# DINT-NSDI24/DINT

Measured on NVIDIA H100. Metric: committed txns/sec (lock_fasst), higher is better.
Workload: dtype u32

## Files before the change

### dint_b200/csrc/engine.cu

```cuda
#include <cmath>
#include <cstdio>
#include <cstdlib>
#include <cstring>
#include <string>
#include <algorithm>
#include <chrono>
#include <type_traits>
#include <vector>
#include <cerrno>
#include <fcntl.h>
#include <sys/stat.h>
#include <unistd.h>

#include "../../include/dint_b200.h"
#include "kernels.cuh"
#include "route.cuh"
#include "kv.cuh"
#include "clients.cuh"
#include "txn_clients.cuh"
#include "image.cuh"
#include "reshard.cuh"
#include "rebuild.cuh"

using namespace dint;

static thread_local std::string g_last_error;
static int set_err(int code, const char* what, cudaError_t ce = cudaSuccess) {
  char buf[1024];
  if (ce != cudaSuccess) snprintf(buf, sizeof buf, "%s: %s", what, cudaGetErrorString(ce));
  else snprintf(buf, sizeof buf, "%s", what);
  g_last_error = buf;
  return code;
}
template <typename... Args>
static int set_errf(int code, const char* fmt, Args... args) {
  char buf[1024];
  snprintf(buf, sizeof buf, fmt, args...);
  return set_err(code, buf);
}
#define CU(call)                                                              \
  do {                                                                        \
    cudaError_t _e = (call);                                                  \
    if (_e != cudaSuccess) return set_err(_e == cudaErrorMemoryAllocation ? DINT_ENOMEM : DINT_EIO, #call, _e); \
  } while (0)

static const uint32_t kMsgSize[DINT_NUM_KINDS] = {6, 9, 53, 53, 55, 23};
static const uint32_t kLogEntry[DINT_NUM_KINDS] = {0, 0, 56, 0, 64, 32};
static const uint32_t kValSize[DINT_NUM_KINDS] = {0, 0, 0, 40, 40, 8};

constexpr int kExecStoreEbpf = DINT_NUM_KINDS;
constexpr int kExecTatpEbpf = DINT_NUM_KINDS + 1;
constexpr int kExecSmallbankEbpf = DINT_NUM_KINDS + 2;

template <class F>
static int with_kind(int kind, F&& f) {
  switch (kind) {
    case DINT_LOCK2PL: return f(std::integral_constant<int, K_LOCK2PL>{});
    case DINT_FASST: return f(std::integral_constant<int, K_FASST>{});
    case DINT_LOG: return f(std::integral_constant<int, K_LOG>{});
    case DINT_STORE: return f(std::integral_constant<int, K_STORE>{});
    case DINT_TATP: return f(std::integral_constant<int, K_TATP>{});
    case DINT_SMALLBANK: return f(std::integral_constant<int, K_SMALLBANK>{});
    case kExecStoreEbpf: return f(std::integral_constant<int, K_STORE_EBPF>{});
    case kExecTatpEbpf: return f(std::integral_constant<int, K_TATP_EBPF>{});
    case kExecSmallbankEbpf: return f(std::integral_constant<int, K_SMALLBANK_EBPF>{});
  }
  return set_err(DINT_EINVAL, "bad kind");
}

struct StepTarget {
  uint32_t seg_tiles;
  uint64_t seg_resp[kMaxShards];
  bool pad_ok;
  const uint32_t* skip;
};

enum { KT_CLASSIFY = 0, KT_LOGSCAN, KT_APPLY, KT_ORDERED, KT_LOAD, KT_NUM };
static const char* kKernelNames[KT_NUM] = {"k_classify", "k_log_scan", "k_apply", "k_ordered", "k_kv_load"};

struct EvPair { cudaEvent_t a, b; int which; };
constexpr int kHostBufs = 4;
struct HostRing {
  struct Buf { uint8_t* p = nullptr; size_t cap = 0; };
  Buf in[kHostBufs], aux[kHostBufs], out[kHostBufs];
  cudaEvent_t h2d[kHostBufs]{}, released[kHostBufs]{}, ready[kHostBufs]{}, d2h[kHostBufs]{};
  cudaStream_t s_in = nullptr, s_out = nullptr;
  uint32_t sets = 0;
};

struct dint_engine {
  int kind = 0;
  int device = 0;
  dint_cfg cfg{};
  uint32_t msg = 0;
  uint32_t chunk = 0;
  uint32_t max_tiles = 0;
  bool has_log = false;
  Ctx ctx{};
  std::vector<void*> allocs;
  cudaStream_t stream = nullptr;
  HostRing ring;
  uint32_t host_chunk = 0;
  bool plain_launches = false;
  uint32_t host_min_slice = 0;
  bool host_ramp_up = true;
  unsigned long long* h_counters = nullptr;
  unsigned long long* h_kvcnt = nullptr;
  cudaEvent_t ev_kvcnt = nullptr;
  int coop_grid = 0;
  int sms = 0;
  int grid_classify = 0, grid_apply = 0;
  uint32_t smem_stage = 0;
  uint64_t total_groups = 0;
  uint32_t* d_flags[2] = {nullptr, nullptr};
  uint32_t* d_grp[2] = {nullptr, nullptr};
  uint64_t chunk_seq = 0;
  uint32_t prev_n = 0;
  bool ord_pending = false;
  uint8_t* ord_resp = nullptr;
  const uint8_t* ord_req = nullptr;
  uint32_t ord_tile0 = 0;
  uint32_t smem_classify = 0;
  uint32_t* d_nc = nullptr;
  uint32_t* d_route = nullptr;
  uint32_t route_tiles = 0;
  uint32_t* d_route2 = nullptr;
  uint32_t route_desc_tiles = 0, route_seq = 0;
  int grid_route = 0;
  uint8_t* hot_arena = nullptr;
  size_t hot_bytes = 0;
  bool use_window = false;
  cudaAccessPolicyWindow window{};
  dint_stats stats{};
  uint32_t profiling = 0;
  std::vector<EvPair> ev_pool;
  size_t ev_used = 0;
  double kt_ms[KT_NUM] = {0};
  uint64_t kt_n[KT_NUM] = {0};
  KvHost kv[kMaxTables];
};

static bool sbe_on(const dint_engine* e) { return e->kind == DINT_SMALLBANK && e->ctx.ecache; }
static int exec_kind(const dint_engine* e) {
  return e->ctx.tchain ? kExecTatpEbpf : sbe_on(e) ? kExecSmallbankEbpf : e->ctx.ecache ? kExecStoreEbpf : e->kind;
}

template <typename T>
static int dalloc(dint_engine* e, T** p, size_t count, bool zero = true) {
  size_t bytes = count * sizeof(T);
  if (bytes == 0) bytes = sizeof(T);
  void* q = nullptr;
  CU(cudaMalloc(&q, bytes));
  e->allocs.push_back(q);
  if (zero) CU(cudaMemsetAsync(q, 0, bytes, e->stream));
  *p = (T*)q;
  return DINT_OK;
}

static int prof_flush(dint_engine* e) {
  for (size_t i = 0; i < e->ev_used; i++) {
    float ms = 0;
    CU(cudaEventSynchronize(e->ev_pool[i].b));
    CU(cudaEventElapsedTime(&ms, e->ev_pool[i].a, e->ev_pool[i].b));
    e->kt_ms[e->ev_pool[i].which] += ms;
    e->kt_n[e->ev_pool[i].which]++;
  }
  e->ev_used = 0;
  return DINT_OK;
}
struct ProfScope {
  dint_engine* e; cudaStream_t s; EvPair* p = nullptr;
  ProfScope(dint_engine* e_, cudaStream_t s_, int which) : e(e_), s(s_) {
    e->stats.kernel_launches++;
    if (!((e->profiling >> which) & 1u)) return;
    if (e->ev_used == e->ev_pool.size()) {
      if (e->ev_pool.size() >= 8192) { prof_flush(e); }
      else {
        EvPair np{}; cudaEventCreate(&np.a); cudaEventCreate(&np.b);
        e->ev_pool.push_back(np);
      }
    }
    p = &e->ev_pool[e->ev_used++];
    p->which = which;
    cudaEventRecord(p->a, s);
  }
  ~ProfScope() { if (p) cudaEventRecord(p->b, s); }
};

template <typename... Args>
static cudaError_t launch_ex(dint_engine* e, void (*kern)(Args...), int grid, int block, size_t smem, cudaStream_t s,
                             bool coop, Args... args) {
  cudaLaunchConfig_t cfg{};
  cfg.gridDim = dim3(grid < 1 ? 1 : grid);
  cfg.blockDim = dim3(block);
  cfg.dynamicSmemBytes = smem;
  cfg.stream = s;
  cudaLaunchAttribute at[3];
  int na = 0;
  if (coop) { at[na].id = cudaLaunchAttributeCooperative; at[na].val.cooperative = 1; na++; }
  if (e->use_window) { at[na].id = cudaLaunchAttributeAccessPolicyWindow; at[na].val.accessPolicyWindow = e->window; na++; }
  cfg.attrs = at;
  cfg.numAttrs = na;
  return cudaLaunchKernelEx(&cfg, kern, args...);
}

template <int KIND>
static int launch_chunk_t(dint_engine* e, const Ctx& c, cudaStream_t s) {
  {
    ProfScope ps(e, s, KT_CLASSIFY);
    int want = (int)c.n_tiles, clr = (int)((c.prev_n + 4 * kTile - 1) / (4 * kTile));
    if (clr > want) want = clr;
    int grid = (want < e->grid_classify && !c.ord_pending) ? want : e->grid_classify;
    if (c.n == 0 && e->sms > 0 && grid > 8 * e->sms) grid = 8 * e->sms;
    CU(launch_ex(e, k_classify<KIND>, grid, kTile, e->smem_classify, s, false, c));
  }
  if (c.n == 0) { CU(cudaGetLastError()); return DINT_OK; }
  if (kHasLog<KIND>) {
    ProfScope ps(e, s, KT_LOGSCAN);
    k_log_scan<<<1, kThreads, 0, s>>>(c);
  }
  {
    ProfScope ps(e, s, KT_APPLY);
    int grid = (int)c.n_tiles < e->grid_apply ? (int)c.n_tiles : e->grid_apply;
    CU(launch_ex(e, k_apply<KIND>, grid, kTile, e->smem_stage, s, false, c));
  }
  if ((KIND == K_TATP || KIND == K_TATP_EBPF) && c.n > c.ring_n) {
    int grid = (int)((c.ring_n + kThreads - 1) / kThreads);
    if (e->sms > 0 && grid > 4 * e->sms) grid = 4 * e->sms;
    k_log_vals<<<grid, kThreads, 0, s>>>(c);
    e->stats.kernel_launches++;
  }
  if (KIND != K_LOG) {
    ProfScope ps(e, s, KT_ORDERED);
    Ctx f = c;
    f.nc_ord = c.nc_cur;
    f.ord_resp = c.resp;
    f.ord_req = c.req;
    f.ord_tile0 = c.tile0;
    f.coop_launch = e->plain_launches ? 0u : 1u;
    int g3 = e->coop_grid;
    if (e->plain_launches && e->sms > 0) {
      const int per = g3 / e->sms;
      g3 = (per > 1 ? per - 1 : 1) * e->sms;
    }
    CU(launch_ex(e, k_ordered<KIND>, g3, kThreads, 0, s, !e->plain_launches, f));
  }
  CU(cudaGetLastError());
  return DINT_OK;
}

static int launch_chunk(dint_engine* e, const Ctx& c, cudaStream_t s) {
  return with_kind(exec_kind(e), [&](auto k) { return launch_chunk_t<decltype(k)::value>(e, c, s); });
}

template <int KIND>
static int grids_for(dint_engine* e) {
  int per_sm = 0, sms = 0;
  CU(cudaDeviceGetAttribute(&sms, cudaDevAttrMultiProcessorCount, e->device));
  e->sms = sms;
  e->grid_route = 4 * sms;
  e->smem_stage = Stage<Wire<KIND>::MSG>::N * Stage<Wire<KIND>::MSG>::BYTES;
  if (e->smem_stage > 48 * 1024) {
    CU(cudaFuncSetAttribute(k_classify<KIND>, cudaFuncAttributeMaxDynamicSharedMemorySize, (int)e->smem_stage));
    CU(cudaFuncSetAttribute(k_apply<KIND>, cudaFuncAttributeMaxDynamicSharedMemorySize, (int)e->smem_stage));
  }
  e->smem_classify = e->smem_stage;
  if (KIND != K_LOG && (kTile / 32) * OrdSlice<KIND>::BYTES > e->smem_classify) e->smem_classify = (kTile / 32) * OrdSlice<KIND>::BYTES;
  CU(cudaOccupancyMaxActiveBlocksPerMultiprocessor(&per_sm, k_classify<KIND>, kTile, e->smem_classify));
  if (per_sm < 1) return set_err(DINT_EIO, "k_classify cannot be resident");
  e->grid_classify = per_sm * sms;
  CU(cudaOccupancyMaxActiveBlocksPerMultiprocessor(&per_sm, k_apply<KIND>, kTile, e->smem_stage));
  if (per_sm < 1) return set_err(DINT_EIO, "k_apply cannot be resident");
  e->grid_apply = per_sm * sms;
  if (KIND == K_LOG) { e->coop_grid = 1; return DINT_OK; }
  CU(cudaOccupancyMaxActiveBlocksPerMultiprocessor(&per_sm, k_ordered<KIND>, kThreads, 0));
  if (per_sm < 1) return set_err(DINT_EIO, "k_ordered cannot be resident");
  if (per_sm > 4) per_sm = 4;
  e->coop_grid = per_sm * sms;
  return DINT_OK;
}

static void fill_chunk_ctx(dint_engine* e, Ctx& c, const StepTarget* tgt) {
  const int cur = (int)(e->chunk_seq & 1);
  c.grp = e->d_grp[cur];
  c.grp_prev = e->d_grp[cur ^ 1];
  c.flags = e->d_flags[cur];
  c.flags_prev = e->d_flags[cur ^ 1];
  c.prev_n = e->prev_n;
  c.clear_set = (uint64_t)(c.flags_mask + 1) / 256 <= e->prev_n ? 1u : 0u;
  c.nc_cur = e->d_nc + 4 * cur;
  c.nc_ord = e->d_nc + 4 * (cur ^ 1);
  c.ord_pending = e->ord_pending ? 1u : 0u;
  c.ord_resp = e->ord_resp;
  c.ord_req = e->ord_req;
  c.ord_tile0 = e->ord_tile0;
  if (tgt) {
    c.seg_tiles = tgt->seg_tiles;
    c.pad_ok = tgt->pad_ok ? 1u : 0u;
    c.skip = tgt->skip;
    for (int i = 0; i < kMaxShards; i++) c.seg_resp[i] = tgt->seg_resp[i];
  }
}

static int submit_chunk(dint_engine* e, const uint8_t* req, uint32_t n, uint8_t* resp, cudaStream_t s, uint32_t tile0 = 0,
                        const StepTarget* tgt = nullptr) {
  Ctx c = e->ctx;
  c.n = n;
  c.n_tiles = (n + kTile - 1) / kTile;
  c.req = req;
  c.resp = resp;
  c.tile0 = tile0;
  fill_chunk_ctx(e, c, tgt);
  int rc = launch_chunk(e, c, s);
// ... 185 lines not shown
  }
  e->route_seq = e->route_seq % 255u + 1u;
  if (e->route_seq == 1)
    CU(cudaMemsetAsync(e->d_route2, 0, 64 + (size_t)(e->route_desc_tiles + e->route_desc_tiles / 32 + 1) * 4 * sizeof(unsigned long long), s));
  RouteArgs b = a;
  b.done = e->d_route2;
  b.ticket = e->d_route2 + 1;
  b.totals = e->d_route2 + 4;
  b.desc = (unsigned long long*)(e->d_route2 + 16);
  b.gdesc = b.desc + (size_t)e->route_desc_tiles * 4;
  b.seq = e->route_seq;
  if (CUDART_VERSION >= 11000 && RT::SMEM > 48 * 1024) CU(cudaFuncSetAttribute(k_route_dispatch<KIND>, cudaFuncAttributeMaxDynamicSharedMemorySize, (int)RT::SMEM));
  int grid = (int)b.n_tiles < e->grid_route ? (int)b.n_tiles : e->grid_route;
  if (grid < 1) grid = 1;
  k_route_dispatch<KIND><<<grid, kThreads, RT::SMEM, s>>>(e->ctx, b);
  CU(cudaGetLastError());
  return DINT_OK;
}
template <int MSG>
static int route_combine_t(dint_engine* e, const RouteArgs& a, cudaStream_t s) {
  using RT = RTile<MSG>;
  int grid = (int)a.n_tiles;
  if (grid > e->grid_route) grid = e->grid_route;
  k_route_combine<MSG><<<grid, kThreads, RT::SMEM, s>>>(a);
  CU(cudaGetLastError());
  return DINT_OK;
}
static uint32_t route_tile_records(const dint_engine* e) { return e->msg <= 12 ? kThreads * 8u : (uint32_t)kThreads; }

extern "C" {

uint32_t dint_msg_size(int kind) { return (kind >= 0 && kind < DINT_NUM_KINDS) ? kMsgSize[kind] : 0; }
uint32_t dint_log_entry_size(int kind) { return (kind >= 0 && kind < DINT_NUM_KINDS) ? kLogEntry[kind] : 0; }
const char* dint_last_error(void) { return g_last_error.c_str(); }
uint64_t dint_test_fasthash64(uint64_t x, int len) { return len == 4 ? fasthash64_u32((uint32_t)x) : fasthash64_u64(x); }
uint32_t dint_test_fastmod(uint64_t n, uint32_t d) { FastMod f = make_fastmod(d); return fast_mod(n, f); }
int dint_test_rebuild_source(uint64_t key, uint32_t G, uint32_t lost_mask) {
  return G == 0 || G > kMaxShards ? -1 : rebuild_source((uint32_t)(key % G), G, lost_mask);
}
uint32_t dint_test_host_slices(uint64_t n, uint32_t min_slice, uint32_t max_slice, int ramp_up, uint32_t* out, uint32_t cap) {
  HostSlices sched(n, min_slice, max_slice, ramp_up != 0);
  uint32_t k = 0;
  for (uint32_t cn; (cn = sched.next()) != 0; k++)
    if (k < cap) out[k] = cn;
  return k;
}

void dint_default_cfg(int kind, dint_cfg* cfg) {
  memset(cfg, 0, sizeof *cfg);
  cfg->lock_slots = 36000000u;
  cfg->log_ring = 1000000u;
  cfg->subs_sizing = (kind == DINT_TATP) ? 7000000u : 2000000u;
  cfg->subs_populate = cfg->subs_sizing;
  cfg->accts_sizing = 24000000u;
  cfg->accts_populate = cfg->accts_sizing;
  cfg->n_shards = 1;
  cfg->shard_id = 0;
  cfg->chunk = 1u << 20;
}

void* dint_host_alloc(size_t bytes) {
  void* p = nullptr;
  if (cudaHostAlloc(&p, bytes ? bytes : 1, cudaHostAllocDefault) != cudaSuccess) { cudaGetLastError(); return nullptr; }
  return p;
}
void dint_host_free(void* p) { if (p) cudaFreeHost(p); }

void dint_destroy(dint_engine* e) {
  if (!e) return;
  cudaSetDevice(e->device);
  cudaDeviceSynchronize();
  for (void* p : e->allocs) cudaFree(p);
  if (e->d_route) cudaFree(e->d_route);
  if (e->d_route2) cudaFree(e->d_route2);
  if (e->h_counters) cudaFreeHost(e->h_counters);
  if (e->h_kvcnt) cudaFreeHost(e->h_kvcnt);
  if (e->ev_kvcnt) cudaEventDestroy(e->ev_kvcnt);
  for (auto& ep : e->ev_pool) { cudaEventDestroy(ep.a); cudaEventDestroy(ep.b); }
  HostRing& R = e->ring;
  for (int i = 0; i < kHostBufs; i++) {
    for (HostRing::Buf* b : {&R.in[i], &R.aux[i], &R.out[i]}) cudaFree(b->p);
    for (cudaEvent_t ev : {R.h2d[i], R.released[i], R.ready[i], R.d2h[i]}) if (ev) cudaEventDestroy(ev);
  }
  for (cudaStream_t s : {e->stream, R.s_in, R.s_out}) if (s) cudaStreamDestroy(s);
  delete e;
}

static int create_impl(dint_engine* e) {
  const dint_cfg& cf = e->cfg;
  Ctx& c = e->ctx;
  CU(cudaSetDevice(e->device));
  CU(cudaStreamCreateWithFlags(&e->stream, cudaStreamNonBlocking));
  HostRing& R = e->ring;
  for (cudaStream_t* s : {&R.s_in, &R.s_out}) CU(cudaStreamCreateWithFlags(s, cudaStreamNonBlocking));
  for (int i = 0; i < kHostBufs; i++)
    for (cudaEvent_t* ev : {&R.h2d[i], &R.released[i], &R.ready[i], &R.d2h[i]}) CU(cudaEventCreateWithFlags(ev, cudaEventDisableTiming));
  c.n_shards = cf.n_shards;
  c.shard_id = cf.shard_id;
  c.shard_div = make_fastmod(cf.n_shards);
  c.slot_mod = make_fastmod(cf.lock_slots);
  c.ring_n = cf.log_ring ? cf.log_ring : 1;

  uint64_t groups = 0;
  auto local_groups = [&](uint64_t global) { return (global + cf.n_shards - 1) / cf.n_shards; };
  int rc;
  switch (e->kind) {
    case DINT_LOCK2PL:
      groups = local_groups(cf.lock_slots);
      if ((rc = dalloc(e, &c.cnt2, groups))) return rc;
      break;
    case DINT_FASST:
      groups = local_groups(cf.lock_slots);
      if ((rc = dalloc(e, &c.ver, groups))) return rc;
      break;
    case DINT_LOG:
      groups = 0;
      break;
    default:
      if ((rc = kv_create_tables(e->kind, cf, c, e->kv, &groups,
                                 [&](void** p, size_t bytes) -> int {
                                   uint8_t* q = nullptr;
                                   int r = dalloc(e, &q, bytes);
                                   *p = q;
                                   return r;
                                 },
                                 (cf.flags & DINT_CFG_TATP_EBPF) != 0)))
        return rc == DINT_EINVAL ? set_err(rc, "bad KV configuration") : rc;
      break;
  }
  e->total_groups = groups;
  if (groups >= 0xffffffffULL) return set_err(DINT_EINVAL, "too many groups");
  if ((cf.flags & DINT_CFG_LOCK_HOLDER_KEYS) && (rc = dalloc(e, &c.holder, groups))) return rc;
  if (cf.flags & DINT_CFG_STORE_EBPF_MASK) {
    c.ecache_variant = (cf.flags & DINT_CFG_STORE_EBPF_MASK) >> 1;
    if ((rc = dalloc(e, &c.ecache, groups * kEcSetBytes))) return rc;
    if ((rc = dalloc(e, &c.ecache_stats, EC_NSTATS))) return rc;
  }
  if (cf.flags & DINT_CFG_TATP_EBPF) {
    const uint64_t buckets = groups / 4;
    for (uint32_t t = 0; t < c.n_tables; t++) c.tbkt_mod[t] = make_fastmod(e->kv[t].hash_size);
    c.tpool_cap = (uint32_t)(buckets + buckets / 2 + 4096);
    if ((rc = dalloc(e, &c.ecache, buckets * kEcSetBytes))) return rc;
    if ((rc = dalloc(e, &c.ecache_stats, EC_NSTATS_TATP))) return rc;
    if ((rc = dalloc(e, &c.tchain, buckets))) return rc;
    if ((rc = dalloc(e, &c.tpool, (size_t)c.tpool_cap * kTeEntBytes))) return rc;
    if ((rc = dalloc(e, &c.tpool_top, 1))) return rc;
  }
  if (cf.flags & DINT_CFG_SMALLBANK_EBPF) {
    for (uint32_t t = 0; t < c.n_tables; t++) c.tbkt_mod[t] = make_fastmod(e->kv[t].hash_size);
    if ((rc = dalloc(e, &c.ecache, groups / 4 * kSbeSetBytes))) return rc;
    if ((rc = dalloc(e, &c.ecache_stats, SBE_NSTATS))) return rc;
  }
  {
    uint32_t fl = 25;
    while (fl > 10 && (1ULL << (fl - 1)) >= groups * 2 + 2048) fl--;
    c.flags_mask = (1u << fl) - 1;
    const size_t set_bytes = (size_t)4 << (fl - 3);
    const size_t lock_bytes = (e->kind == DINT_FASST) ? (((groups + 31) / 32) * 4 + 255) / 256 * 256 : 0;
    e->hot_bytes = 2 * set_bytes + lock_bytes;
    if ((rc = dalloc(e, &e->hot_arena, e->hot_bytes))) return rc;
    e->d_flags[0] = (uint32_t*)e->hot_arena;
    e->d_flags[1] = (uint32_t*)(e->hot_arena + set_bytes);
    if (lock_bytes) c.lockbits = (uint32_t*)(e->hot_arena + 2 * set_bytes);
    int max_persist = 0, max_win = 0;
    cudaDeviceGetAttribute(&max_persist, cudaDevAttrMaxPersistingL2CacheSize, e->device);
    cudaDeviceGetAttribute(&max_win, cudaDevAttrMaxAccessPolicyWindowSize, e->device);
    if (max_persist > 0 && max_win > 0) {
      size_t want = e->hot_bytes < (size_t)max_persist ? e->hot_bytes : (size_t)max_persist;
      if (cudaDeviceSetLimit(cudaLimitPersistingL2CacheSize, want) == cudaSuccess) {
        e->window.base_ptr = e->hot_arena;
        e->window.num_bytes = e->hot_bytes < (size_t)max_win ? e->hot_bytes : (size_t)max_win;
        e->window.hitRatio = (float)((double)want / (double)e->window.num_bytes > 1.0 ? 1.0 : (double)want / (double)e->window.num_bytes);
        e->window.hitProp = cudaAccessPropertyPersisting;
        e->window.missProp = cudaAccessPropertyStreaming;
        e->use_window = true;
// ... 2725 lines not shown
```

### dint_b200/csrc/kernels.cuh

```cuda
#pragma once
#include <cooperative_groups.h>
#include "engine.cuh"

namespace dint {
namespace cg = cooperative_groups;

DINT_D uint32_t lane_id() { return threadIdx.x & 31; }
DINT_D uint32_t warp_id() { return threadIdx.x >> 5; }

DINT_D uint32_t tile_rank(bool flag, uint32_t* scratch, uint32_t& total) {
  uint32_t bal = __ballot_sync(0xffffffffu, flag);
  uint32_t in_warp = __popc(bal & ((1u << lane_id()) - 1u));
  if (lane_id() == 0) scratch[warp_id()] = __popc(bal);
  __syncthreads();
  uint32_t off = 0, tot = 0;
#pragma unroll
  for (int w = 0; w < kTile / 32; w++) {
    uint32_t v = scratch[w];
    if (w < (int)warp_id()) off += v;
    tot += v;
  }
  __syncthreads();
  total = tot;
  return off + in_warp;
// ... 106 lines not shown
}
template <int KIND>
__global__ void __launch_bounds__(kThreads) k_route_owner(const Ctx c, const uint8_t* req, uint32_t n, uint8_t* owner) {
  const uint32_t i = blockIdx.x * kThreads + threadIdx.x;
  if (i < n) owner[i] = (uint8_t)route_owner_of<KIND>(c, req + (size_t)i * Wire<KIND>::MSG);
}

constexpr int kMaxShards = 8;
__global__ void __launch_bounds__(kThreads) k_exact_count(const uint8_t* owner, uint32_t n, uint32_t world, uint32_t* tilecnt) {
  __shared__ uint32_t cnt[kMaxShards];
  if (threadIdx.x < kMaxShards) cnt[threadIdx.x] = 0;
  __syncthreads();
  const uint32_t i = blockIdx.x * kThreads + threadIdx.x;
  const uint32_t o = i < n ? owner[i] : 0xffu;
  const uint32_t peers = __match_any_sync(0xffffffffu, o);
  if (o < world && (int)lane_id() == __ffs(peers) - 1) atomicAdd(&cnt[o], (uint32_t)__popc(peers));
  __syncthreads();
  if (threadIdx.x < world) tilecnt[(size_t)threadIdx.x * gridDim.x + blockIdx.x] = cnt[threadIdx.x];
}
__global__ void __launch_bounds__(kThreads) k_exact_scan(uint32_t* tilecnt, uint32_t n_tiles, uint32_t* totals) {
  __shared__ uint32_t wsum[kThreads / 32];
  uint32_t* row = tilecnt + (size_t)blockIdx.x * n_tiles;
  const uint32_t total = cta_exclusive_scan<uint32_t>(row, row, n_tiles, 0u, wsum);
  if (threadIdx.x == 0) totals[blockIdx.x] = total;
}
template <int MSG>
__global__ void __launch_bounds__(kThreads) k_exact_scatter(const uint8_t* req, const uint8_t* owner, uint32_t n, uint32_t world,
                                                            const uint32_t* tilebase, const uint32_t* totals, uint8_t* out,
                                                            uint32_t* perm) {
  __shared__ uint32_t wcnt[kThreads / 32][kMaxShards];
  const uint32_t i = blockIdx.x * kThreads + threadIdx.x;
  if (threadIdx.x < (kThreads / 32) * kMaxShards) ((uint32_t*)wcnt)[threadIdx.x] = 0;
  __syncthreads();
  const uint32_t o = i < n ? owner[i] : 0xffu;
  const uint32_t peers = __match_any_sync(0xffffffffu, o);
  const uint32_t before = __popc(peers & ((1u << lane_id()) - 1u));
  if (o < world && before == 0) wcnt[warp_id()][o] = __popc(peers);
  __syncthreads();
  if (o < world) {
    uint32_t pos = tilebase[(size_t)o * gridDim.x + blockIdx.x] + before;
    for (uint32_t w = 0; w < warp_id(); w++) pos += wcnt[w][o];
    for (uint32_t q = 0; q < o; q++) pos += totals[q];
    copy_record<MSG>(out + (size_t)pos * MSG, req + (size_t)i * MSG);
    perm[pos] = i;
  }
}
struct PeerPtrs { uint64_t p[kMaxShards]; };

__global__ void k_p2p_signal(PeerPtrs sig, uint32_t world, uint32_t me, uint32_t epoch) {
  if (threadIdx.x < world) {
    __threadfence_system();
    volatile uint32_t* flag = (volatile uint32_t*)sig.p[threadIdx.x] + me;
    asm volatile("st.release.sys.global.u32 [%0], %1;" ::"l"(flag), "r"(epoch) : "memory");
  }
}
constexpr uint32_t kSigOverflow = 0x80000000u;
__global__ void k_p2p_wait(const uint32_t* my_sig, uint32_t world, uint32_t epoch, uint32_t* timeout, uint32_t* bad) {
  if (threadIdx.x < world) {
    const long long t0 = clock64();
    uint32_t v;
    do {
      asm volatile("ld.acquire.sys.global.u32 %0, [%1];" : "=r"(v) : "l"(my_sig + threadIdx.x) : "memory");
      if (clock64() - t0 > 8000000000LL) { atomicExch(timeout, 1u); break; }
    } while ((int32_t)((v & ~kSigOverflow) - epoch) < 0);
    if (bad && (v & kSigOverflow) && (v & ~kSigOverflow) == epoch) atomicCAS(bad, 0u, epoch);
  }
  __syncthreads();
  __threadfence_system();
}

template <int MSG>
__global__ void __launch_bounds__(kThreads) k_exact_unpermute(const uint8_t* sorted, const uint32_t* perm, uint32_t n, uint8_t* out) {
  const uint32_t pos = blockIdx.x * kThreads + threadIdx.x;
  if (pos >= n) return;
  const uint32_t idx = perm[pos];
  if (idx == 0xffffffffu) return;
  copy_record<MSG>(out + (size_t)idx * MSG, sorted + (size_t)pos * MSG);
}

template <int KIND> struct OrdSlice {
  static constexpr uint32_t BYTES = kBucketCap * (FastReplay<KIND>::ok ? (8 + 8 + 4) : 8);
};
template <int KIND> DINT_D void ordered_buckets(const Ctx& c, uint8_t* scratch);

template <int KIND>
__global__ void __launch_bounds__(kTile) k_classify(const Ctx c) {
  using W = Wire<KIND>;
  constexpr uint32_t NS = Stage<W::MSG>::N;
  extern __shared__ __align__(128) uint8_t smem[];
  __shared__ uint64_t full[kStages];
  __shared__ uint32_t scratch[kTile / 32];
  if (c.skip && __ldcg(c.skip)) return;
  if (threadIdx.x == 0) {
    for (int s = 0; s < kStages; s++) mbar_init(&full[s], 1);
    if (blockIdx.x == 0) { c.nc_cur[0] = 0; c.nc_cur[1] = 0; c.nc_ord[2] = 0; }
  }
  __syncthreads();
  const bool do_ord = c.ord_pending && c.nc_ord[0] != 0 && c.nc_ord[1] == 0;
  const bool ord_first = (blockIdx.x & 1u) != 0;
  if (do_ord && ord_first) {
    ordered_buckets<KIND>(c, smem);
    __syncthreads();
  }
  const TileIter it = tile_iter(c.n_tiles);
  if (threadIdx.x == 0)
    for (uint32_t i = 0; i < NS && i < it.n_my; i++) issue_tile_load<W::MSG>(c, smem, full, it, i);

  if (c.clear_set) {
    uint4* f4 = (uint4*)c.flags_prev;
    const uint32_t n4 = (c.flags_mask + 1) / 32;
    for (uint32_t i = blockIdx.x * kTile + threadIdx.x; i < n4; i += gridDim.x * kTile) f4[i] = make_uint4(0, 0, 0, 0);
  }
  for (uint32_t i = blockIdx.x * kTile + threadIdx.x; !c.clear_set && i < c.prev_n; i += 4 * gridDim.x * kTile) {
    uint32_t g[4];
#pragma unroll
    for (int u = 0; u < 4; u++) {
      const uint32_t j = i + u * gridDim.x * kTile;
      g[u] = j < c.prev_n ? __ldcg(&c.grp_prev[j]) : kNoGroup;
    }
#pragma unroll
    for (int u = 0; u < 4; u++)
      if (g[u] != kNoGroup) c.flags_prev[flag_word(c, g[u])] = 0;
  }

  uint32_t pend_old = 0, pend_test = 0, pend_sh = 0;
  uint32_t* pend_w = nullptr;
  bool saw_writer = false;
  for (uint32_t i = 0; it.has(i); i++) {
    if (threadIdx.x == 0 && i && i + NS - 1 < it.n_my) issue_tile_load<W::MSG>(c, smem, full, it, i + NS - 1);
    uint32_t first, cnt;
    const uint8_t* tile = acquire_tile<W::MSG>(c, smem, full, it, i, first, cnt);
    const bool valid = threadIdx.x < cnt;
    bool is_log = false;
    uint32_t new_old = 0, new_test = 0, new_sh = 0;
    uint32_t* new_w = nullptr;
    if (valid) {
      const uint8_t* rec = tile + threadIdx.x * W::MSG;
      TypeInfo ti = (c.pad_ok && rec[W::TYPE] == kPadType) ? TypeInfo{0, false, false} : type_info<KIND>(rec);
      uint32_t g = kNoGroup;
      if (!ti.invalid && ti.mask) {
        g = key_info<KIND>(c, rec).grp;
        if (g != kNoGroup) {
          uint32_t* w = &c.flags[flag_word(c, g)];
          const uint32_t sh = flag_shift(g);
          if (ti.mask == C_RA) {
            atomicOr(w, F_R << sh);
          } else {
            const uint32_t bits = ((ti.mask & C_RA) ? F_R : 0u) | ((ti.mask & C_WA) ? F_WA : 0u) | ((ti.mask & C_WL) ? F_WL : 0u);
            saw_writer = true;
            new_old = atomicOr(w, bits << sh);
            new_test = ((ti.mask & C_WA) ? F_WA : 0u) | ((ti.mask & C_WL) ? F_WL : 0u);
            new_w = w;
            new_sh = sh;
          }
        }
      }
      c.grp[first + threadIdx.x] = g;
      is_log = !ti.invalid && ti.is_log;
    }
    if (pend_w && ((pend_old >> pend_sh) & pend_test)) atomicOr(pend_w, F_W2 << pend_sh);
    pend_old = new_old; pend_test = new_test; pend_sh = new_sh; pend_w = new_w;
    if (kHasLog<KIND>) {
      uint32_t total;
      (void)tile_rank(is_log, scratch, total);
      if (threadIdx.x == 0) c.log_tilecnt[it.tile(i)] = total;
    } else {
      __syncthreads();
    }
  }
  if (pend_w && ((pend_old >> pend_sh) & pend_test)) atomicOr(pend_w, F_W2 << pend_sh);
  if (__syncthreads_or(saw_writer ? 1 : 0) && threadIdx.x == 0) atomicOr(&c.nc_cur[2], 1u);
  if (do_ord && !ord_first) {
    __syncthreads();
    ordered_buckets<KIND>(c, smem);
  }
}

__global__ void __launch_bounds__(kThreads) k_log_scan(const Ctx c) {
  if (c.skip && __ldcg(c.skip)) return;
  __shared__ uint32_t wsum[kThreads / 32];
  const unsigned long long end =
      cta_exclusive_scan<unsigned long long>(c.log_tilecnt, c.log_tilebase, c.n_tiles, threadIdx.x == 0 ? c.log_total[0] : 0ull, wsum);
  if (threadIdx.x == 0) {
    c.log_total[1] = end;
    c.log_total[0] = end;
  }
}

__global__ void __launch_bounds__(kThreads) k_log_vals(const Ctx c) {
  using W = Wire<K_TATP>;
  if (c.skip && __ldcg(c.skip)) return;
  const unsigned long long base = c.log_tilebase[0], end = c.log_total[1];
  if (end - base <= c.ring_n) return;
  for (unsigned long long ord = end - c.ring_n + blockIdx.x * kThreads + threadIdx.x; ord < end; ord += (unsigned long long)gridDim.x * kThreads) {
    if (c.log_src[ord - base] & 1u) continue;
    for (unsigned long long o = ord; o >= base + c.ring_n;) {
      o -= c.ring_n;
      const uint32_t s = c.log_src[o - base];
      if (s & 1u) {
        const uint8_t* src = c.req + (size_t)(s >> 1) * W::MSG + W::VAL;
        uint8_t* e = c.ring + (size_t)(ord % c.ring_n) * W::LOGENT + 16;
        for (int b = 0; b < 40; b++) e[b] = src[b];
        break;
      }
    }
  }
}

template <int KIND>
__global__ void __launch_bounds__(kTile) k_apply(const Ctx c) {
  using W = Wire<KIND>;
  constexpr uint32_t NS = Stage<W::MSG>::N;
  extern __shared__ __align__(128) uint8_t smem[];
  __shared__ uint64_t full[kStages];
  __shared__ uint32_t scratch2[2][kTile / 32];
  constexpr bool kGrpFromK1 = (KIND == K_LOCK2PL || KIND == K_FASST);
  if (c.skip && __ldcg(c.skip)) return;
  if (threadIdx.x == 0)
    for (int s = 0; s < kStages; s++) mbar_init(&full[s], 1);
  __syncthreads();
  const TileIter it = tile_iter(c.n_tiles);
  if (threadIdx.x == 0)
    for (uint32_t i = 0; i < NS && i < it.n_my; i++) issue_tile_load<W::MSG>(c, smem, full, it, i);
  const bool chunk_has_writer = c.nc_cur[2] != 0;

  for (uint32_t i = 0; it.has(i); i++) {
    uint32_t* scratch = scratch2[i & 1];
    uint32_t g_k1 = kNoGroup;
    if (kGrpFromK1) {
      const uint32_t idx = it.tile(i) * kTile + threadIdx.x;
      if (idx < c.n) g_k1 = __ldcg(&c.grp[idx]);
    }
    if (threadIdx.x == 0 && i && i + NS - 1 < it.n_my) {
      asm volatile("cp.async.bulk.wait_group.read 0;" ::: "memory");
      issue_tile_load<W::MSG>(c, smem, full, it, i + NS - 1);
    }
    uint32_t first, cnt;
    uint8_t* tile = acquire_tile<W::MSG>(c, smem, full, it, i, first, cnt);
    const uint32_t t = it.tile(i);
    const bool valid = threadIdx.x < cnt;
    uint8_t* rec = tile + threadIdx.x * W::MSG;
    TypeInfo ti{0, false, false};
    KeyInfo ki{0, 0, kNoGroup};
    Pre<KIND> pf;
    bool listed = false;
    const bool pad = valid && c.pad_ok && rec[W::TYPE] == kPadType;
    if (valid && !pad) {
      ti = type_info<KIND>(rec);
      if (!ti.invalid && ti.mask) {
        if (kGrpFromK1) ki.grp = g_k1; else ki = key_info<KIND>(c, rec);
        if (ki.grp == kNoGroup) ti.invalid = true;
      }
    }
    {
      const bool active = valid && !ti.invalid && ti.mask;
      pf = prefetch_coop<KIND>(c, rec, ki, ti, active);
      if (active && chunk_has_writer) {
        const uint32_t f = (__ldcg(&c.flags[flag_word(c, ki.grp)]) >> flag_shift(ki.grp)) & 15u;
        listed = ((ti.mask & C_RA) && (f & F_WA)) || ((ti.mask & C_WA) && (f & (F_R | F_W2))) ||
                 ((ti.mask & C_WL) && (f & F_W2));
// ... 468 lines not shown
```

### dint_b200/engine.py

```python
import ctypes as C
import os

import numpy as np

from . import _build
from .wire import MSG_SIZE, LOG_ENTRY_SIZE, KIND_NAMES

DINT_OK, DINT_EPROTO = 0, -71
DINT_CFG_LOCK_HOLDER_KEYS = 1
DINT_CFG_STORE_EBPF_WB_BLOOM, DINT_CFG_STORE_EBPF_WB, DINT_CFG_STORE_EBPF_WT = 1 << 1, 2 << 1, 3 << 1
DINT_CFG_STORE_EBPF_MASK = 3 << 1
STORE_EBPF_VARIANTS = {"wb_bloom": DINT_CFG_STORE_EBPF_WB_BLOOM, "wb": DINT_CFG_STORE_EBPF_WB, "wt": DINT_CFG_STORE_EBPF_WT}
STORE_CACHE_ENTRY_BYTES = 232
STORE_CACHE_STATS = ("hits", "bloom_negatives", "table", "write_backs", "installs")
DINT_CFG_TATP_EBPF = 1 << 3
TATP_CHAIN_REC = np.dtype([("key", "<u8", (4,)), ("ver", "<u4", (4,)), ("valid", "u1", (4,)), ("val", "u1", (4, 40))])
TATP_CACHE_STATS = STORE_CACHE_STATS + ("allocated", "reused", "freed", "failed")
DINT_CFG_SMALLBANK_EBPF = 1 << 4
SMALLBANK_CACHE_ENTRY_BYTES = 96
SMALLBANK_CACHE_STATS = ("hits", "table", "write_backs", "installs")


class DintCfg(C.Structure):
    _fields_ = [("lock_slots", C.c_uint32), ("log_ring", C.c_uint32), ("subs_sizing", C.c_uint32),
# ... 441 lines not shown

    def store_cache_stats(self):
        out = (C.c_uint64 * 5)()
        rc = lib().dint_store_cache_stats(self.h, out)
        if rc != 0:
            raise DintError(rc, "dint_store_cache_stats")
        return {k: int(out[i]) for i, k in enumerate(STORE_CACHE_STATS)}

    def tatp_cache_set(self, table, bucket):
        out = np.zeros(STORE_CACHE_ENTRY_BYTES, dtype=np.uint8)
        rc = lib().dint_tatp_cache_set(self.h, table, bucket, out.ctypes.data)
        if rc != 0:
            raise DintError(rc, "dint_tatp_cache_set")
        return out

    def tatp_chain(self, table, bucket, max_entries=64):
        out = np.zeros(max_entries, dtype=TATP_CHAIN_REC)
        n = C.c_uint32(0)
        rc = lib().dint_tatp_chain(self.h, table, bucket, out.ctypes.data, max_entries, C.byref(n))
        if rc != 0:
            raise DintError(rc, "dint_tatp_chain")
        if n.value > max_entries:
            return self.tatp_chain(table, bucket, n.value)
        return out[:n.value]

    def tatp_cache_stats(self):
        out = (C.c_uint64 * 9)()
        rc = lib().dint_tatp_cache_stats(self.h, out)
        if rc != 0:
            raise DintError(rc, "dint_tatp_cache_stats")
        return {k: int(out[i]) for i, k in enumerate(TATP_CACHE_STATS)}

    def smallbank_cache_set(self, table, bucket):
        out = np.zeros(SMALLBANK_CACHE_ENTRY_BYTES, dtype=np.uint8)
        rc = lib().dint_smallbank_cache_set(self.h, table, bucket, out.ctypes.data)
        if rc != 0:
            raise DintError(rc, "dint_smallbank_cache_set")
        return out

    def smallbank_cache_stats(self):
        out = (C.c_uint64 * 4)()
        rc = lib().dint_smallbank_cache_stats(self.h, out)
        if rc != 0:
            raise DintError(rc, "dint_smallbank_cache_stats")
        return {k: int(out[i]) for i, k in enumerate(SMALLBANK_CACHE_STATS)}

    def lock_slot(self, table, key):
        return lib().dint_lock_slot(self.h, table, key)

    def lock_state(self, table, slot):
        out = (C.c_uint32 * 2)()
        rc = lib().dint_lock_state(self.h, table, slot, out)
        if rc != 0:
            raise DintError(rc, "dint_lock_state")
        return out[0], out[1]

    def lock_holder(self, table, slot):
        out = C.c_uint64(0)
        rc = lib().dint_lock_holder(self.h, table, slot, C.byref(out))
        if rc != 0:
            raise DintError(rc, "dint_lock_holder")
        return out.value

    def dump_log(self):
        es = LOG_ENTRY_SIZE[self.kind]
        n = self.cfg.log_ring
        out = np.zeros((n, es), dtype=np.uint8)
        appended = C.c_uint64(0)
        rc = lib().dint_dump_log(self.h, out.ctypes.data, C.byref(appended))
        if rc != 0:
            raise DintError(rc, "dint_dump_log")
        return out, appended.value

    def stats(self):
        s = DintStats()
        rc = lib().dint_get_stats(self.h, C.byref(s))
        if rc != 0:
            raise DintError(rc, "dint_get_stats")
        return {k: getattr(s, k) for k, _ in DintStats._fields_ if k != "reserved"}

    def reset_stats(self):
        lib().dint_reset_stats(self.h)

    PROF_CLASSIFY, PROF_LOG_SCAN, PROF_APPLY, PROF_ORDERED, PROF_LOAD = 1, 2, 4, 8, 16

    def profile(self, enable=True):
        rc = lib().dint_profile(self.h, int(enable))
        if rc != 0:
            raise DintError(rc, "dint_profile")

    def kernel_times(self):
        arr = (DintKernelTime * 16)()
        k = lib().dint_kernel_times(self.h, arr, 16)
        return {arr[i].name.decode(): (arr[i].launches, arr[i].total_ms) for i in range(max(k, 0))}


class GpuClients:

    def __init__(self, engine, n_clients, seed=20230, n_keys=24_000_000, zipf_theta=0.0, read_pct=80, set_pct=0,
                 store_subscribers=2_000_000, store_hot=False):
        self.engine, self.n, self.kind = engine, n_clients, engine.kind
        self.msg = MSG_SIZE[self.kind]
        cfg = DintClientsCfg(n_clients=n_clients, n_keys=n_keys, seed=seed, zipf_theta=zipf_theta, read_pct=read_pct,
                             set_pct=set_pct, store_subscribers=store_subscribers, store_hot=1 if store_hot else 0)
        h = C.c_void_p()
        rc = lib().dint_clients_create_cfg(engine.h, C.byref(cfg), C.byref(h))
        if rc != 0:
            raise DintError(rc, "dint_clients_create_cfg")
        self.h = h

    def run(self, rounds, stream=None):
        if stream is None:
            import torch
            stream = torch.cuda.current_stream().cuda_stream
        rc = lib().dint_clients_run(self.h, rounds, C.c_void_p(stream) if stream else None)
        if rc != 0:
            raise DintError(rc, "dint_clients_run")

    def stats(self):
        out = (C.c_uint64 * 6)()
        rc = lib().dint_clients_stats_all(self.h, out)
        if rc != 0:
            raise DintError(rc, "dint_clients_stats_all")
        keys = ["requests", "committed", "validation_aborts", "lock_rejects", "not_exist", "rounds"]
        return dict(zip(keys, [int(x) for x in out]))

    def peek(self):
        rq = np.empty(self.n * self.msg, dtype=np.uint8)
        rs = np.empty(self.n * self.msg, dtype=np.uint8)
        rc = lib().dint_clients_peek(self.h, rq.ctypes.data, rs.ctypes.data)
        if rc != 0:
            raise DintError(rc, "dint_clients_peek")
        return rq, rs

    def close(self):
        if getattr(self, "h", None):
            lib().dint_clients_destroy(self.h)
            self.h = None

    def __enter__(self):
        return self

    def __exit__(self, *a):
        self.close()

    def __del__(self):
        try:
            self.close()
        except Exception:
            pass


class GpuCluster:

    def __init__(self, kind, n_shards, devices=None, max_batch=0, populate=False, **cfg_over):
        self.kind, self.msg, self.G = kind, MSG_SIZE[kind], n_shards
        cfg = self.cfg = default_cfg(kind, **cfg_over)
        dv = (C.c_int * n_shards)(*devices) if devices is not None else None
        h = C.c_void_p()
        rc = lib().dint_cluster_create(kind, C.byref(cfg), n_shards, dv, max_batch, C.byref(h))
        if rc != 0:
            raise DintError(rc, f"dint_cluster_create({KIND_NAMES[kind]}, {n_shards})")
        self.h = h
        if populate:
            rc = lib().dint_cluster_populate(self.h)
            if rc != 0:
                raise DintError(rc, "dint_cluster_populate")
# ... 235 lines not shown
```

Baseline: 322.4 million.

## Move previous-chunk flag clearing to a side stream overlapping apply

For FASST and 2PL lock kinds, clearing of the previous chunk's conflict flags is taken out of k_classify and moved into a new k_retire kernel. That kernel runs on a side stream forked after classify and joined before k_ordered, so it can overlap log scan and apply. The aim is to shorten classify's critical path and its grid sizing, which was driven by prev_n. In exchange it adds an extra launch plus event record and wait per chunk, and concurrent kernels may contend for SMs.

```diff
diff --git a/dint_b200/csrc/engine.cu b/dint_b200/csrc/engine.cu
--- a/dint_b200/csrc/engine.cu
+++ b/dint_b200/csrc/engine.cu
@@ -75,8 +75,8 @@
   const uint32_t* skip;
 };
 
-enum { KT_CLASSIFY = 0, KT_LOGSCAN, KT_APPLY, KT_ORDERED, KT_LOAD, KT_NUM };
-static const char* kKernelNames[KT_NUM] = {"k_classify", "k_log_scan", "k_apply", "k_ordered", "k_kv_load"};
+enum { KT_CLASSIFY = 0, KT_LOGSCAN, KT_APPLY, KT_ORDERED, KT_LOAD, KT_RETIRE, KT_NUM };
+static const char* kKernelNames[KT_NUM] = {"k_classify", "k_log_scan", "k_apply", "k_ordered", "k_kv_load", "k_retire"};
 
 struct EvPair { cudaEvent_t a, b; int which; };
 constexpr int kHostBufs = 4;
@@ -99,6 +99,8 @@
   Ctx ctx{};
   std::vector<void*> allocs;
   cudaStream_t stream = nullptr;
+  cudaStream_t side = nullptr;
+  cudaEvent_t ev_fork = nullptr, ev_join = nullptr;
   HostRing ring;
   uint32_t host_chunk = 0;
   bool plain_launches = false;
@@ -208,13 +210,15 @@
 static int launch_chunk_t(dint_engine* e, const Ctx& c, cudaStream_t s) {
   {
     ProfScope ps(e, s, KT_CLASSIFY);
-    int want = (int)c.n_tiles, clr = (int)((c.prev_n + 4 * kTile - 1) / (4 * kTile));
+    int want = (int)c.n_tiles, clr = kRetireBesideApply<KIND> ? 0 : (int)((c.prev_n + 4 * kTile - 1) / (4 * kTile));
     if (clr > want) want = clr;
     int grid = (want < e->grid_classify && !c.ord_pending) ? want : e->grid_classify;
     if (c.n == 0 && e->sms > 0 && grid > 8 * e->sms) grid = 8 * e->sms;
     CU(launch_ex(e, k_classify<KIND>, grid, kTile, e->smem_classify, s, false, c));
   }
   if (c.n == 0) { CU(cudaGetLastError()); return DINT_OK; }
+  const bool retire = kRetireBesideApply<KIND> && c.prev_n > 0;
+  if (retire) CU(cudaEventRecord(e->ev_fork, s));
   if (kHasLog<KIND>) {
     ProfScope ps(e, s, KT_LOGSCAN);
     k_log_scan<<<1, kThreads, 0, s>>>(c);
@@ -223,12 +227,23 @@
     ProfScope ps(e, s, KT_APPLY);
     int grid = (int)c.n_tiles < e->grid_apply ? (int)c.n_tiles : e->grid_apply;
     CU(launch_ex(e, k_apply<KIND>, grid, kTile, e->smem_stage, s, false, c));
+  }
+  if (retire) {
+    CU(cudaStreamWaitEvent(e->side, e->ev_fork, 0));
+    ProfScope ps(e, e->side, KT_RETIRE);
+    int grid = c.clear_set ? (int)((c.flags_mask + 1) / 32 / kThreads) : (int)((c.prev_n + 4 * kThreads - 1) / (4 * kThreads));
+    if (e->sms > 0 && grid > e->sms) grid = e->sms;
+    k_retire<<<grid < 1 ? 1 : grid, kThreads, 0, e->side>>>(c);
   }
   if ((KIND == K_TATP || KIND == K_TATP_EBPF) && c.n > c.ring_n) {
     int grid = (int)((c.ring_n + kThreads - 1) / kThreads);
     if (e->sms > 0 && grid > 4 * e->sms) grid = 4 * e->sms;
     k_log_vals<<<grid, kThreads, 0, s>>>(c);
     e->stats.kernel_launches++;
+  }
+  if (retire) {
+    CU(cudaEventRecord(e->ev_join, e->side));
+    CU(cudaStreamWaitEvent(s, e->ev_join, 0));
   }
   if (KIND != K_LOG) {
     ProfScope ps(e, s, KT_ORDERED);
@@ -580,7 +595,8 @@
     for (HostRing::Buf* b : {&R.in[i], &R.aux[i], &R.out[i]}) cudaFree(b->p);
     for (cudaEvent_t ev : {R.h2d[i], R.released[i], R.ready[i], R.d2h[i]}) if (ev) cudaEventDestroy(ev);
   }
-  for (cudaStream_t s : {e->stream, R.s_in, R.s_out}) if (s) cudaStreamDestroy(s);
+  for (cudaEvent_t ev : {e->ev_fork, e->ev_join}) if (ev) cudaEventDestroy(ev);
+  for (cudaStream_t s : {e->stream, e->side, R.s_in, R.s_out}) if (s) cudaStreamDestroy(s);
   delete e;
 }
 
@@ -589,6 +605,8 @@
   Ctx& c = e->ctx;
   CU(cudaSetDevice(e->device));
   CU(cudaStreamCreateWithFlags(&e->stream, cudaStreamNonBlocking));
+  CU(cudaStreamCreateWithFlags(&e->side, cudaStreamNonBlocking));
+  for (cudaEvent_t* ev : {&e->ev_fork, &e->ev_join}) CU(cudaEventCreateWithFlags(ev, cudaEventDisableTiming));
   HostRing& R = e->ring;
   for (cudaStream_t* s : {&R.s_in, &R.s_out}) CU(cudaStreamCreateWithFlags(s, cudaStreamNonBlocking));
   for (int i = 0; i < kHostBufs; i++)
diff --git a/dint_b200/csrc/kernels.cuh b/dint_b200/csrc/kernels.cuh
--- a/dint_b200/csrc/kernels.cuh
+++ b/dint_b200/csrc/kernels.cuh
@@ -212,6 +212,7 @@
   static constexpr uint32_t BYTES = kBucketCap * (FastReplay<KIND>::ok ? (8 + 8 + 4) : 8);
 };
 template <int KIND> DINT_D void ordered_buckets(const Ctx& c, uint8_t* scratch);
+template <int KIND> constexpr bool kRetireBesideApply = KIND == K_FASST || KIND == K_LOCK2PL;
 
 template <int KIND>
 __global__ void __launch_bounds__(kTile) k_classify(const Ctx c) {
@@ -236,12 +237,12 @@
   if (threadIdx.x == 0)
     for (uint32_t i = 0; i < NS && i < it.n_my; i++) issue_tile_load<W::MSG>(c, smem, full, it, i);
 
-  if (c.clear_set) {
+  if (!kRetireBesideApply<KIND> && c.clear_set) {
     uint4* f4 = (uint4*)c.flags_prev;
     const uint32_t n4 = (c.flags_mask + 1) / 32;
     for (uint32_t i = blockIdx.x * kTile + threadIdx.x; i < n4; i += gridDim.x * kTile) f4[i] = make_uint4(0, 0, 0, 0);
   }
-  for (uint32_t i = blockIdx.x * kTile + threadIdx.x; !c.clear_set && i < c.prev_n; i += 4 * gridDim.x * kTile) {
+  for (uint32_t i = blockIdx.x * kTile + threadIdx.x; !kRetireBesideApply<KIND> && !c.clear_set && i < c.prev_n; i += 4 * gridDim.x * kTile) {
     uint32_t g[4];
 #pragma unroll
     for (int u = 0; u < 4; u++) {
@@ -306,6 +307,27 @@
   }
 }
 
+__global__ void __launch_bounds__(kThreads) k_retire(const Ctx c) {
+  if (c.skip && __ldcg(c.skip)) return;
+  if (c.clear_set) {
+    uint4* f4 = (uint4*)c.flags_prev;
+    const uint32_t n4 = (c.flags_mask + 1) / 32;
+    for (uint32_t i = blockIdx.x * kThreads + threadIdx.x; i < n4; i += gridDim.x * kThreads) f4[i] = make_uint4(0, 0, 0, 0);
+    return;
+  }
+  for (uint32_t i = blockIdx.x * kThreads + threadIdx.x; i < c.prev_n; i += 4 * gridDim.x * kThreads) {
+    uint32_t g[4];
+#pragma unroll
+    for (int u = 0; u < 4; u++) {
+      const uint32_t j = i + u * gridDim.x * kThreads;
+      g[u] = j < c.prev_n ? __ldcg(&c.grp_prev[j]) : kNoGroup;
+    }
+#pragma unroll
+    for (int u = 0; u < 4; u++)
+      if (g[u] != kNoGroup) c.flags_prev[flag_word(c, g[u])] = 0;
+  }
+}
+
 __global__ void __launch_bounds__(kThreads) k_log_scan(const Ctx c) {
   if (c.skip && __ldcg(c.skip)) return;
   __shared__ uint32_t wsum[kThreads / 32];
diff --git a/dint_b200/engine.py b/dint_b200/engine.py
--- a/dint_b200/engine.py
+++ b/dint_b200/engine.py
@@ -547,7 +547,7 @@
     def reset_stats(self):
         lib().dint_reset_stats(self.h)
 
-    PROF_CLASSIFY, PROF_LOG_SCAN, PROF_APPLY, PROF_ORDERED, PROF_LOAD = 1, 2, 4, 8, 16
+    PROF_CLASSIFY, PROF_LOG_SCAN, PROF_APPLY, PROF_ORDERED, PROF_LOAD, PROF_RETIRE = 1, 2, 4, 8, 16, 32
 
     def profile(self, enable=True):
         rc = lib().dint_profile(self.h, int(enable))
```

Measured after the change: 327.4 million, median of 6. +1.5%, better.
